# ChainSafe/halo2-verifier

Hardware: AMD Instinct MI355X
Metric: proofs verified/sec (BN254, k=14) (higher is better)
Workload: dtype u32 limbs (254-bit prime-field integers)

## Files before the change

### halo2_verifier_amd/csrc/bn254.hip.h

```cpp
#pragma once
#include <hip/hip_runtime.h>
#include <stdint.h>

#define H2V_HD __host__ __device__ inline
#define H2V_FN __host__ __device__ inline __attribute__((noinline))

namespace h2v {

#define H2V_LIMBS 9
#define H2V_LIMB_BITS 29
#define H2V_LIMB_MASK 0x1fffffffu

struct FqParams {
    static constexpr uint32_t INV29 = 0x04866389u;
    H2V_HD static constexpr uint32_t P(int i) {
        constexpr uint32_t p[8] = {0xd87cfd47u, 0x3c208c16u, 0x6871ca8du, 0x97816a91u, 0x8181585du, 0xb85045b6u, 0xe131a029u, 0x30644e72u};
        return p[i];
    }
    H2V_HD static constexpr uint32_t P29(int i) {
        constexpr uint32_t v[9] = {0x187cfd47u, 0x010460b6u, 0x1c72a34fu, 0x02d522d0u, 0x1585d978u, 0x02db40c0u, 0x00a6e141u, 0x0e5c2634u, 0x0030644eu};
        return v[i];
    }
    H2V_HD static constexpr uint32_t ONE(int i) {
        constexpr uint32_t v[9] = {0x157ccc21u, 0x141c2758u, 0x185230d3u, 0x014c0419u, 0x0aa36fb9u, 0x1d4240ceu, 0x11d54c07u, 0x052ac7a8u, 0x000dc836u};
        return v[i];
    }
    H2V_HD static constexpr uint32_t R2(int i) {
        constexpr uint32_t v[9] = {0x059bac10u, 0x0d1503a3u, 0x018016b8u, 0x10ab0ca8u, 0x02632639u, 0x02c0169fu, 0x169bfd53u, 0x11869d4cu, 0x002a11a6u};
        return v[i];
    }
    H2V_HD static constexpr uint32_t M256(int i) {
        constexpr uint32_t v[9] = {0x0f6b5c04u, 0x08ead878u, 0x1645525du, 0x1aefe9cdu, 0x09d605edu, 0x0483a115u, 0x0d08508bu, 0x0dba4804u, 0x001982b4u};
        return v[i];
    }
    H2V_HD static constexpr uint32_t K266(int i) {
// ... 323 lines not shown
        r.v[8] = (uint32_t)acc;
        return r;
    }
    __host__ __device__ __forceinline__ Fp sqr_inl() const {
        uint64_t acc = 0;
        uint32_t m[9], d[9];
        Fp r;
#pragma unroll
        for (int i = 0; i < 9; ++i) d[i] = v[i] << 1;
#pragma unroll
        for (int k = 0; k < 9; ++k) {
#pragma unroll
            for (int i = 0; 2 * i < k; ++i) acc += (uint64_t)d[i] * v[k - i];
            if (k % 2 == 0) acc += (uint64_t)v[k / 2] * v[k / 2];
#pragma unroll
            for (int i = 0; i < k; ++i) acc += (uint64_t)m[i] * PR::P29(k - i);
            m[k] = ((uint32_t)acc * PR::INV29) & H2V_LIMB_MASK;
            acc += (uint64_t)m[k] * PR::P29(0);
            acc >>= 29;
        }
#pragma unroll
        for (int k = 9; k < 17; ++k) {
#pragma unroll
            for (int i = k - 8; 2 * i < k; ++i) acc += (uint64_t)d[i] * v[k - i];
            if (k % 2 == 0) acc += (uint64_t)v[k / 2] * v[k / 2];
#pragma unroll
            for (int i = k - 8; i <= 8; ++i) acc += (uint64_t)m[i] * PR::P29(k - i);
            r.v[k - 9] = (uint32_t)acc & H2V_LIMB_MASK;
            acc >>= 29;
        }
        r.v[8] = (uint32_t)acc;
        return r;
    }
    H2V_FN static Fp mul(Fp a, Fp b) { return mul_inl(a, b); }
    H2V_FN static Fp sqr_fn(Fp a) { return a.sqr_inl(); }
    H2V_HD Fp operator*(const Fp& b) const { return mul(*this, b); }
    H2V_HD Fp sqr() const { return sqr_fn(*this); }

    H2V_HD static Fp from_raw(const uint32_t raw[8]) { Fp t; pack29(t.v, raw); return mul(t, r2()); }
    H2V_HD static Fp from_raw_unreduced(const uint32_t raw[8]) { return from_raw(raw); }
    H2V_HD static Fp from_mont256(const uint32_t m[8]) { Fp t, k; pack29(t.v, m); for (int i = 0; i < 9; ++i) k.v[i] = PR::K266(i); return mul(t, k); }
    H2V_HD void to_raw(uint32_t out[8]) const {
        Fp o = zero(); o.v[0] = 1;
        Fp r = mul(*this, o);
        uint32_t c[9]; r.canonical(c);
        unpack29(out, c);
    }
    H2V_HD static Fp from_u32(uint32_t x) { uint32_t raw[8] = {x, 0, 0, 0, 0, 0, 0, 0}; return from_raw(raw); }

    H2V_HD static bool from_bytes(const uint8_t b[32], Fp& out) {
        uint32_t raw[8];
        for (int i = 0; i < 8; ++i) raw[i] = (uint32_t)b[4 * i] | ((uint32_t)b[4 * i + 1] << 8) | ((uint32_t)b[4 * i + 2] << 16) | ((uint32_t)b[4 * i + 3] << 24);
        if (geq_p(raw)) return false;
        out = from_raw(raw);
        return true;
    }
    H2V_HD void to_bytes(uint8_t b[32]) const {
        uint32_t raw[8]; to_raw(raw);
        for (int i = 0; i < 8; ++i) { b[4 * i] = (uint8_t)raw[i]; b[4 * i + 1] = (uint8_t)(raw[i] >> 8); b[4 * i + 2] = (uint8_t)(raw[i] >> 16); b[4 * i + 3] = (uint8_t)(raw[i] >> 24); }
    }
    H2V_HD static Fp from_uniform_words(const uint32_t w[16]) {
        Fp lo = from_raw(w), hi = from_raw(w + 8), m256;
        for (int i = 0; i < 9; ++i) m256.v[i] = PR::M256(i);
        return lo + hi * m256;
    }

    H2V_FN Fp pow_u32(uint32_t e) const {
        Fp r = one();
// ... 42 lines not shown
```

### halo2_verifier_amd/csrc/curve.hip.h

```cpp
#pragma once
#include "bn254.hip.h"

namespace h2v {

static constexpr uint8_t G1_FLAG_IDENTITY = 0x80;
static constexpr uint8_t G1_FLAG_SIGN = 0x40;

struct G1A {
    Fq x, y;
    H2V_HD bool is_identity() const { return x.is_zero() && y.is_zero(); }
    H2V_HD static G1A identity() { G1A p; p.x = Fq::zero(); p.y = Fq::zero(); return p; }
    H2V_HD bool on_curve() const {
        if (is_identity()) return true;
        Fq three = Fq::from_u32(3);
        return y.sqr() == x.sqr() * x + three;
    }
};

struct G1J {
    Fq X, Y, Z;
    H2V_HD static G1J identity() { G1J p; p.X = Fq::zero(); p.Y = Fq::one(); p.Z = Fq::zero(); return p; }
    H2V_HD bool is_identity() const { return Z.is_zero(); }
    H2V_HD static G1J from_affine(const G1A& a) {
        if (a.is_identity()) return identity();
        G1J p; p.X = a.x; p.Y = a.y; p.Z = Fq::one(); return p;
    }
    H2V_HD G1J neg() const { G1J r = *this; r.Y = Y.neg(); return r; }
};

H2V_FN G1J g1_dbl(const G1J& p);
#define H2V_M(a, b) Fq::mul_inl((a), (b))
#define H2V_S(a) (a).sqr_inl()
__host__ __device__ __forceinline__ Fq g1_minus_eight() {
    const Fq k = {{0x1d9096cdu, 0x022be75eu, 0x12c66350u, 0x1e1f47a4u, 0x0b760e9fu, 0x1e7fbbcfu, 0x134a4383u, 0x01be3557u, 0x0022eb3au}};
    return k;
}
__host__ __device__ __forceinline__ G1J g1_dbl_inl(const G1J& p) {
    if (p.is_identity()) return p;
    const Fq A = H2V_S(p.X), B = H2V_S(p.Y), XB = H2V_M(p.X, B), C = H2V_S(B);
    const Fq E = Fq::lazy_add2(A, A), F = H2V_S(E), D = Fq::lazy_dbl(Fq::lazy_dbl(XB));
    int64_t acc[9];
#pragma unroll
    for (int l = 0; l < 9; ++l) acc[l] = (int64_t)F.v[l] + (int64_t)Fq::KP29(9, l) - 2 * (int64_t)D.v[l];
    G1J r;
    r.X = Fq::from_wide(acc);
    r.Y = Fq::dot2_inl(E, Fq::lazy_sub(D, r.X), C, g1_minus_eight());
    r.Z = H2V_M(Fq::lazy_dbl(p.Y), p.Z);
    return r;
}

__host__ __device__ __forceinline__ bool g1_madd_fast(G1J& acc, const G1A& q) {
    if (q.is_identity()) return true;
    if (acc.is_identity()) { acc.X = q.x; acc.Y = q.y; acc.Z = Fq::one(); return true; }
    const Fq Z1Z1 = H2V_S(acc.Z);
    const Fq U2 = H2V_M(q.x, Z1Z1), S2 = H2V_M(H2V_M(q.y, acc.Z), Z1Z1);
    const Fq H = Fq::lazy_sub(U2, acc.X), H2 = Fq::lazy_dbl(H), I = H2V_S(H2);
    if (I.is_zero()) return false;
    const Fq B = Fq::lazy_neg2(acc.Y), rr = Fq::lazy_add2(B, S2);
    const Fq X3 = Fq::dot2_inl(rr, rr, I, Fq::template lazy_lin<8, 1, 2>(H, acc.X));
    const Fq W = Fq::dot2_inl(rr, acc.X, H, B);
    acc.Y = Fq::dot2_inl(I, W, rr, Fq::lazy_neg(X3));
    acc.Z = H2V_M(acc.Z, H2);
    acc.X = X3;
    return true;
}
__host__ __device__ __forceinline__ bool g1_add_fast(G1J& acc, const G1J& q) {
    if (q.is_identity()) return true;
    if (acc.is_identity()) { acc.X = q.X; acc.Y = q.Y; acc.Z = q.Z; return true; }
    const Fq Z1Z1 = H2V_S(acc.Z), Z2Z2 = H2V_S(q.Z);
    const Fq U1 = H2V_M(acc.X, Z2Z2), U2 = H2V_M(q.X, Z1Z1);
    const Fq H = Fq::lazy_sub(U2, U1), H2 = Fq::lazy_dbl(H), I = H2V_S(H2);
    if (I.is_zero()) return false;
    const Fq S1 = H2V_M(H2V_M(acc.Y, q.Z), Z2Z2), S2 = H2V_M(H2V_M(q.Y, acc.Z), Z1Z1);
    const Fq B = Fq::lazy_neg2(S1), rr = Fq::lazy_add2(B, S2);
    const Fq X3 = Fq::dot2_inl(rr, rr, I, Fq::template lazy_lin<8, 1, 2>(H, U1));
    const Fq W = Fq::dot2_inl(rr, U1, H, B);
    acc.Y = Fq::dot2_inl(I, W, rr, Fq::lazy_neg(X3));
    acc.Z = H2V_M(H2V_M(acc.Z, q.Z), H2);
    acc.X = X3;
    return true;
}
__host__ __device__ __forceinline__ G1J g1_add_inl(const G1J& p, const G1J& q) {
    G1J r = p;
    if (g1_add_fast(r, q)) return r;
    const Fq Z1Z1 = H2V_S(p.Z), Z2Z2 = H2V_S(q.Z);
    const Fq S1 = H2V_M(H2V_M(p.Y, q.Z), Z2Z2), S2 = H2V_M(H2V_M(q.Y, p.Z), Z1Z1);
    if (S1 == S2) return g1_dbl(r);
    return G1J::identity();
}

__host__ __device__ __forceinline__ G1J g1_add_affine_inl(const G1J& p, const G1A& q) {
    G1J r = p;
    if (g1_madd_fast(r, q)) return r;
    const Fq Z1Z1 = H2V_S(p.Z);
    const Fq S2 = H2V_M(H2V_M(q.y, p.Z), Z1Z1);
    if (p.Y == S2) return g1_dbl(r);
    return G1J::identity();
}

H2V_FN G1J g1_dbl(const G1J& p) { return g1_dbl_inl(p); }
__host__ __device__ __forceinline__ Fq g1_beta_times(const Fq& x) {
    const Fq beta = {{0x18ccb791u, 0x175b1c3au, 0x0b83d6e2u, 0x0e8ed071u, 0x1282bee2u, 0x04220e84u, 0x1fe4017fu, 0x15084d4au, 0x00169119u}};
    return Fq::mul_inl(x, beta);
}
__host__ __device__ __forceinline__ G1A g1_phi(const G1A& p) { G1A r; r.x = g1_beta_times(p.x); r.y = p.y; return r; }
H2V_FN G1J g1_add(const G1J& p, const G1J& q) { return g1_add_inl(p, q); }
H2V_FN G1J g1_add_affine(const G1J& p, const G1A& q) { return g1_add_affine_inl(p, q); }

H2V_FN G1A g1_to_affine(const G1J& p) {
    if (p.is_identity()) return G1A::identity();
    Fq zi = p.Z.inv(), zi2 = zi.sqr();
    G1A a; a.x = p.X * zi2; a.y = p.Y * zi2 * zi;
    return a;
}

struct FqSqrtSchedule { uint8_t op[400]; int n; };
template <int W> constexpr FqSqrtSchedule fq_sqrt_schedule() {
    constexpr uint32_t e[8] = {0xb61f3f52u, 0x4f082305u, 0x5a1c72a3u, 0x65e05aa4u, 0xa0605617u, 0x6e14116du, 0xb84c680au, 0x0c19139cu};
    FqSqrtSchedule s{};
    s.n = 0;
    int i = 255;
    while (i >= 0 && !((e[i >> 5] >> (i & 31)) & 1)) --i;
    while (i >= 0) {
        if (!((e[i >> 5] >> (i & 31)) & 1)) { s.op[s.n++] = 0; --i; continue; }
        int l = i - (W - 1) < 0 ? 0 : i - (W - 1);
        while (!((e[l >> 5] >> (l & 31)) & 1)) ++l;
        uint32_t v = 0;
        for (int k = i; k >= l; --k) { v = (v << 1) | ((e[k >> 5] >> (k & 31)) & 1); s.op[s.n++] = 0; }
        s.op[s.n++] = (uint8_t)((v + 1) / 2);
        i = l - 1;
    }
    return s;
}
template <int W> __host__ __device__ inline __attribute__((noinline)) Fq fq_sqrt_candidate_w(const Fq& a) {
    constexpr FqSqrtSchedule S = fq_sqrt_schedule<W>();
    constexpr int T = 1 << (W - 1);
    Fq t[T];
    t[0] = a;
    const Fq a2 = a.sqr();
#pragma unroll
    for (int k = 1; k < T; ++k) t[k] = t[k - 1] * a2;
    Fq r = Fq::one();
    bool started = false;
#pragma unroll
    for (int k = 0; k < S.n; ++k) {
        if (S.op[k] == 0) { if (started) r = r.sqr(); }
        else { r = started ? r * t[S.op[k] - 1] : t[S.op[k] - 1]; started = true; }
    }
    return r;
}
H2V_FN Fq fq_sqrt_candidate(const Fq& a) { return fq_sqrt_candidate_w<4>(a); }

struct FqSqrtRuns { uint8_t nsq[160]; uint8_t idx[160]; int n; int first; };
template <int W> constexpr FqSqrtRuns fq_sqrt_runs() {
    constexpr FqSqrtSchedule S = fq_sqrt_schedule<W>();
    FqSqrtRuns r{};
    r.n = 0; r.first = -1;
    int pending = 0;
    for (int k = 0; k < S.n; ++k) {
        if (S.op[k] == 0) { if (r.first >= 0) ++pending; continue; }
        if (r.first < 0) { r.first = S.op[k] - 1; continue; }
        r.nsq[r.n] = (uint8_t)pending; r.idx[r.n] = (uint8_t)(S.op[k] - 1); ++r.n; pending = 0;
    }
    if (pending) { r.nsq[r.n] = (uint8_t)pending; r.idx[r.n] = 255; ++r.n; }
    return r;
}
#if defined(__HIPCC__)
__device__ __constant__ const FqSqrtRuns fq_sqrt_runs_w3 = fq_sqrt_runs<3>();
__device__ __forceinline__ Fq fq_sqrt_candidate_loop_w3(const Fq& a) {
    Fq t0 = a;
    const Fq a2 = a.sqr_inl();
    const Fq t1 = Fq::mul_inl(t0, a2), t2 = Fq::mul_inl(t1, a2), t3 = Fq::mul_inl(t2, a2);
    auto pick = [&](uint32_t i) -> Fq {
        Fq s;
#pragma unroll
        for (int l = 0; l < H2V_LIMBS; ++l) s.v[l] = i == 0 ? t0.v[l] : (i == 1 ? t1.v[l] : (i == 2 ? t2.v[l] : t3.v[l]));
        return s;
    };
    Fq r = pick((uint32_t)fq_sqrt_runs_w3.first);
    const int n = fq_sqrt_runs_w3.n;
#pragma unroll 1
    for (int k = 0; k < n; ++k) {
        const uint32_t nsq = fq_sqrt_runs_w3.nsq[k], idx = fq_sqrt_runs_w3.idx[k];
#pragma unroll 1
        for (uint32_t i = 0; i < nsq; ++i) r = r.sqr_inl();
        if (idx == 0u) r = Fq::mul_inl(r, t0);
        else if (idx == 1u) r = Fq::mul_inl(r, t1);
        else if (idx == 2u) r = Fq::mul_inl(r, t2);
        else if (idx == 3u) r = Fq::mul_inl(r, t3);
    }
    return r;
}
#endif

H2V_FN bool g1_decompress(const uint8_t in[32], G1A& out) {
    uint8_t tmp[32];
    for (int i = 0; i < 32; ++i) tmp[i] = in[i];
    bool is_inf = tmp[31] & G1_FLAG_IDENTITY, sign = tmp[31] & G1_FLAG_SIGN;
    tmp[31] &= 0x3f;
    Fq x;
    if (!Fq::from_bytes(tmp, x)) return false;
    if (is_inf) {
        if (!x.is_zero() || sign) return false;
        out = G1A::identity();
        return true;
    }
    Fq rhs = x.sqr() * x + Fq::from_u32(3);
    Fq y = fq_sqrt_candidate(rhs);
    if (y.sqr() != rhs) return false;
    if (y.is_odd() != sign) y = y.neg();
    out.x = x; out.y = y;
    return true;
}

template <int S> __device__ __forceinline__ Fq quad_bcast(const Fq& v) {
    Fq r;
#pragma unroll
    for (int l = 0; l < H2V_LIMBS; ++l) r.v[l] = (uint32_t)__builtin_amdgcn_mov_dpp((int)v.v[l], S * 0x55, 0xf, 0xf, true);
    return r;
}
__device__ __forceinline__ Fq fq_sel(bool c, const Fq& a, const Fq& b) {
    Fq r;
#pragma unroll
    for (int l = 0; l < H2V_LIMBS; ++l) r.v[l] = c ? a.v[l] : b.v[l];
    return r;
}
__device__ __forceinline__ void g1_dbl_quad(G1J& p, uint32_t r) {
    const Fq Y2 = Fq::lazy_dbl(p.Y);
    const Fq p1 = Fq::mul_inl(fq_sel(r == 0, p.X, fq_sel(r == 1, p.Y, Y2)), fq_sel(r == 0, p.X, fq_sel(r == 1, p.Y, p.Z)));
    const Fq A = quad_bcast<0>(p1), B = quad_bcast<1>(p1), Z3 = quad_bcast<2>(p1);
    const Fq E = Fq::lazy_add2(A, A);
    const Fq p2 = Fq::mul_inl(fq_sel(r == 0, B, fq_sel(r == 1, p.X, E)), fq_sel(r == 2, E, B));
    const Fq C = quad_bcast<0>(p2), XB = quad_bcast<1>(p2), F = quad_bcast<2>(p2);
    const Fq D = Fq::lazy_dbl(Fq::lazy_dbl(XB));
    int64_t acc[9];
#pragma unroll
    for (int l = 0; l < 9; ++l) acc[l] = (int64_t)F.v[l] + (int64_t)Fq::KP29(9, l) - 2 * (int64_t)D.v[l];
    p.X = Fq::from_wide(acc);
    p.Y = Fq::dot2_inl(E, Fq::lazy_sub(D, p.X), C, g1_minus_eight());
    p.Z = Z3;
}
template <class Slot> __device__ __forceinline__ G1J msm_horner_quad(const Slot* __restrict__ src, uint32_t items, uint32_t dbl, uint32_t r) {
    G1J acc = src[items - 1].p;
    for (int w = (int)items - 2; w >= 0; --w) {
        const G1J cur = src[w].p;
#pragma unroll 1
        for (uint32_t i = 0; i < dbl; ++i) g1_dbl_quad(acc, r);
        acc = g1_add_inl(acc, cur);
    }
    return acc;
}

}
```

### halo2_verifier_amd/csrc/msm.hip

```cpp
#include "../../include/h2v.h"
#include <hip/hip_ext.h>
#include "batch.h"

namespace h2v {

#define MSM_LDS_SORT_MAX_TERMS 16384u
#define MSM_SORT_THREADS 512u
#define MSM_CHUNK_MIN 16u
#define MSM_CHUNK_MAX 64u
#define MSM_ACC_LANES_PER_ROUND 196608u
#define MSM_CHUNK_SMALL 4u
#define MSM_SHORT_LIST 98304u
__host__ __device__ __forceinline__ uint32_t msm_chunk_len(uint32_t E, uint32_t R) {
    if (E <= MSM_SHORT_LIST) return MSM_CHUNK_SMALL;
    if (E <= R * MSM_CHUNK_MIN) return MSM_CHUNK_MIN;
    const uint32_t k = (uint32_t)(((uint64_t)E + (uint64_t)R * MSM_CHUNK_MAX - 1) / ((uint64_t)R * MSM_CHUNK_MAX));
    const uint32_t c = (uint32_t)(((uint64_t)E + (uint64_t)k * R - 1) / ((uint64_t)k * R));
    return c < MSM_CHUNK_MIN ? MSM_CHUNK_MIN : c;
}
static inline uint32_t msm_accumulate_blocks(size_t max_entries, size_t R) {
    size_t lanes;
    if (max_entries <= R * MSM_CHUNK_MIN)
        lanes = std::max<size_t>((max_entries + MSM_CHUNK_MIN - 1) / MSM_CHUNK_MIN, (std::min<size_t>(max_entries, MSM_SHORT_LIST) + MSM_CHUNK_SMALL - 1) / MSM_CHUNK_SMALL);
    else lanes = (max_entries + R * MSM_CHUNK_MAX - 1) / (R * MSM_CHUNK_MAX) * R;
// ... 638 lines not shown
                                             const uint32_t* __restrict__ lists, G1JSlot* __restrict__ bucket_pts, uint32_t nb, const MsmSeg& g, uint32_t first_block) {
    const uint32_t n_heavy = counts[nb], t = threadIdx.x;
    const uint32_t CH = msm_chunk_len(counts[nb + 1], g.lanes_round);
    for (uint32_t h = blockIdx.x - first_block; h < n_heavy; h += MSM_FIXUP_HEAVY_BLOCKS) {
        const uint32_t b = lists[nb - 1 - h];
        const uint32_t cnt = counts[b], off = msm_bin_start(g, offsets, b);
        const uint32_t i0 = off / CH, i1 = (off + cnt - 1) / CH;
        G1J acc = G1J::identity();
        for (uint32_t i = i0 + t; i <= i1; i += 64) acc = g1_add(acc, msm_piece_src(partial, i, i0, off, CH)->p);
        for (uint32_t d = 32; d > 0; d >>= 1) {
            G1J other;
            uint32_t* dst = reinterpret_cast<uint32_t*>(&other);
            const uint32_t* src = reinterpret_cast<const uint32_t*>(&acc);
#pragma unroll
            for (uint32_t k = 0; k < sizeof(G1J) / 4; ++k) dst[k] = (uint32_t)__shfl_down((int)src[k], d, 64);
            acc = g1_add(acc, other);
        }
        if (t == 0) bucket_pts[b] = acc;
    }
}
__global__ void __launch_bounds__(64) msm_fixup(const uint32_t* __restrict__ counts, const uint32_t* __restrict__ offsets, const G1JSlot* __restrict__ partial,
                                                const uint32_t* __restrict__ lists, G1JSlot* __restrict__ bucket_pts, uint32_t nb, MsmSeg g) {
    __shared__ G1J team_acc[64];
    if (blockIdx.x < MSM_FIXUP_TEAM_BLOCKS) { msm_fixup_team(counts, offsets, partial, lists, bucket_pts, nb, g, team_acc); return; }
    if (blockIdx.x < MSM_FIXUP_TEAM_BLOCKS + MSM_FIXUP_HEAVY_BLOCKS) { msm_fixup_heavy(counts, offsets, partial, lists, bucket_pts, nb, g, MSM_FIXUP_TEAM_BLOCKS); return; }
    const uint32_t k = (blockIdx.x - MSM_FIXUP_TEAM_BLOCKS - MSM_FIXUP_HEAVY_BLOCKS) * blockDim.x + threadIdx.x;
    if (k >= counts[nb + 2]) return;
    const uint32_t b = lists[k];
    const uint32_t cnt = counts[b], off = msm_bin_start(g, offsets, b);
    const uint32_t CH = msm_chunk_len(counts[nb + 1], g.lanes_round);
    const uint32_t i0 = off / CH, i1 = (off + cnt - 1) / CH;
    G1J acc = msm_piece_src(partial, i0, i0, off, CH)->p;
    bool ok = true;
    for (uint32_t i = i0 + 1; i <= i1 && ok; ++i) ok = g1_add_fast(acc, msm_piece_src(partial, i, i0, off, CH)->p);
    if (!ok) { msm_fixup_slow(partial, i0, i1, off, CH, bucket_pts + b); return; }
    bucket_pts[b] = acc;
}
#define MSM_WIN_SLOTS 5
__device__ __noinline__ void g1_add_to(G1J* dst, const G1J* a, const G1J* b) { const G1J x = *a, y = *b; *dst = g1_add_inl(x, y); }
__device__ __noinline__ void g1_dbl_to(G1J* dst, const G1J* a) { const G1J x = *a; *dst = g1_dbl_inl(x); }

__global__ void __launch_bounds__(MSM_WIN_THREADS) msm_window(const G1JSlot* __restrict__ bucket_pts, const uint32_t* __restrict__ counts, G1JSlot* __restrict__ window_sums, MsmPlan p,
                                                              uint32_t n_windows, uint32_t wpw, uint32_t slots) {
    __builtin_amdgcn_s_setprio(3);
    extern __shared__ G1J win_lds[];
    const uint32_t T = blockDim.x / wpw, sub = threadIdx.x / T, t = threadIdx.x % T;
    const uint32_t widx = blockIdx.x * wpw + sub;
    const bool live = widx < n_windows;
    G1J* mine = win_lds + (size_t)sub * slots * T;
    G1J* run = mine + t;
    G1J* sum = mine + T + t;
    G1J* scaled = mine + 2 * T + t;
    G1J* red = mine + 2 * T;
    const uint32_t slice = (p.buckets + T - 1) / T;
    const uint32_t lo = live ? min(p.buckets, t * slice) : 0, hi = live ? min(p.buckets, lo + slice) : 0;
    *run = G1J::identity(); *sum = G1J::identity();
    const G1JSlot* bp = bucket_pts + (size_t)widx * p.buckets;
    const uint32_t* cn = counts + (size_t)widx * p.buckets;
    for (uint32_t b = hi; b > lo; --b) {
        if (cn[b - 1]) g1_add_to(run, run, &bp[b - 1].p);
        g1_add_to(sum, sum, run);
    }
    if ((slice & (slice - 1)) == 0 && T > 1 && slots >= MSM_WIN_SLOTS) {
        G1J* run2 = mine + 3 * T + t;
        G1J* run3 = mine + 4 * T + t;
        if (lo < hi && t > 0) {
            g1_dbl_to(run2, run);
// ... 40 lines not shown
        const uint32_t* src = reinterpret_cast<const uint32_t*>(&mine_sum);
#pragma unroll
        for (uint32_t k = 0; k < sizeof(G1J) / 4; ++k) dst[k] = (uint32_t)__shfl_down((int)src[k], d, 64);
        if ((t & (W - 1)) + d >= W) other = G1J::identity();
        *scaled = other;
        g1_add_to(sum, sum, scaled);
    }
    __syncthreads();
    if ((t & (W - 1)) == 0) red[t >> 6] = *sum;
    __syncthreads();
    if (t == 0) {
        for (uint32_t wv = 1; wv < (T >> 6); ++wv) g1_add_to(&red[0], &red[0], &red[wv]);
        if (live) window_sums[widx] = red[0];
    }
}

__global__ void __launch_bounds__(64) msm_final(const G1JSlot* __restrict__ window_sums, const MsmProblem* __restrict__ prs, uint32_t count, MsmPlan p) {
    __builtin_amdgcn_s_setprio(3);
    const uint32_t t = blockIdx.x * blockDim.x + threadIdx.x, q = t >> 2, r = t & 3u;
    if (q >= count) return;
    G1J acc = G1J::identity();
    if (prs[q].n) acc = msm_horner_quad(window_sums + (size_t)q * p.windows, p.windows, p.c, r);
    if (r == 0) *prs[q].out = acc;
}
__global__ void __launch_bounds__(64) msm_final_parts(const G1JSlot* __restrict__ window_sums, const MsmProblem* __restrict__ prs, uint32_t count, MsmPlan p,
                                                      uint32_t parts, uint32_t wpp, G1JSlot* __restrict__ out, G1JSlot* __restrict__ ready) {
    __builtin_amdgcn_s_setprio(3);
    const uint32_t t = blockIdx.x * blockDim.x + threadIdx.x, quad = t >> 2, r = t & 3u;
    if (quad >= count * parts) return;
    const uint32_t q = quad / parts, j = quad % parts, lo = j * wpp, hi = min(p.windows, lo + wpp);
    G1J acc = G1J::identity();
    if (prs[q].n && lo < hi) acc = msm_horner_quad(window_sums + (size_t)q * p.windows + lo, hi - lo, p.c, r);
    if (r == 0) out[quad] = acc;
    if (r == 0) { ready[quad].p.X = Fq::mul_inl(acc.X, acc.Z); ready[quad].p.Y = acc.Y; }
    if (r == 1) ready[quad].p.Z = Fq::mul_inl(acc.Z.sqr_inl(), acc.Z);
}
__global__ void __launch_bounds__(64) msm_combine_parts(const G1JSlot* __restrict__ pieces, const MsmProblem* __restrict__ prs, uint32_t count, uint32_t parts, uint32_t shift) {
    const uint32_t t = blockIdx.x * blockDim.x + threadIdx.x, q = t >> 2, r = t & 3u;
    if (q >= count) return;
    const G1J acc = msm_horner_quad(pieces + (size_t)q * parts, parts, shift, r);
    if (r == 0) *prs[q].out = acc;
}

__global__ void __launch_bounds__(64) msm_merge_windows(const G1JSlot* __restrict__ sub_sums, const MsmProblem* __restrict__ parents, uint32_t n_parents, uint32_t windows,
                                                        G1JSlot* __restrict__ merged) {
    const uint32_t team = (blockIdx.x * blockDim.x + threadIdx.x) >> 3, r = threadIdx.x & 7u;
    const bool live = team < n_parents * windows;
    const uint32_t q = live ? team / windows : 0, w = live ? team % windows : 0;
    const uint32_t first = parents[q].sub_first, cnt = live ? parents[q].sub_count : 0;
    G1J acc = G1J::identity();
    for (uint32_t k = r; k < cnt; k += 8) acc = g1_add(acc, sub_sums[(size_t)(first + k) * windows + w].p);
    for (uint32_t d = 4; d > 0; d >>= 1) {
        G1J other;
        uint32_t* dst = reinterpret_cast<uint32_t*>(&other);
        const uint32_t* src = reinterpret_cast<const uint32_t*>(&acc);
#pragma unroll
        for (uint32_t k = 0; k < sizeof(G1J) / 4; ++k) dst[k] = (uint32_t)__shfl_down((int)src[k], d, 8);
        acc = g1_add(acc, other);
    }
    if (live && r == 0) merged[(size_t)q * windows + w] = acc;
}

__global__ void msm_set_problems(MsmProblemChunk ch, uint32_t count, MsmProblem* __restrict__ dst) {
    uint32_t i = threadIdx.x;
    if (i < count) dst[i] = ch.p[i];
}

static MsmProblem msm_problem_slice(const MsmProblem& q, uint32_t first, uint32_t len) {
// ... 166 lines not shown
```

### halo2_verifier_amd/csrc/verify_kernels.hip

```cpp
#include "../../include/h2v.h"
#include "batch.h"
#include <atomic>

namespace h2v {

__global__ void __launch_bounds__(64, 4) k_decompress(const uint8_t* __restrict__ proofs, uint32_t proof_len, const uint32_t* __restrict__ point_offsets,
                                                   uint32_t np, uint32_t n_main_points, uint32_t n, G1A* __restrict__ pts, G1A* __restrict__ phi, uint8_t* __restrict__ ycanon,
                                                   int* __restrict__ status) {
    const uint32_t t_raw = blockIdx.x * blockDim.x + threadIdx.x;
    const uint32_t t = min(t_raw, n * np - 1);
    uint32_t p = t / np, slot = t % np;
    const uint4* src = reinterpret_cast<const uint4*>(proofs + (size_t)p * proof_len + point_offsets[slot]);
    const uint4 lo = src[0], hi = src[1];
    uint32_t w[8] = {lo.x, lo.y, lo.z, lo.w, hi.x, hi.y, hi.z, hi.w};
    const bool is_inf = (w[7] >> 24) & G1_FLAG_IDENTITY, sign = (w[7] >> 24) & G1_FLAG_SIGN;
    w[7] &= 0x3fffffffu;
    G1A a = G1A::identity();
    bool ok = !Fq::geq_p(w);
    uint32_t yraw[8] = {0, 0, 0, 0, 0, 0, 0, 0};
    if (ok) {
        const Fq x = Fq::from_raw(w);
        if (is_inf) ok = false;
        else {
            const Fq three = {{FqParams::ONE(0), FqParams::ONE(1), FqParams::ONE(2), FqParams::ONE(3), FqParams::ONE(4), FqParams::ONE(5), FqParams::ONE(6), FqParams::ONE(7), FqParams::ONE(8)}};
            const Fq rhs = x.sqr() * x + (three + three + three);
            Fq y = fq_sqrt_candidate_loop_w3(rhs);
            if (y.sqr() != rhs) ok = false;
            else {
                y.to_raw(yraw);
                uint32_t nz = 0;
#pragma unroll
                for (int i = 0; i < 8; ++i) nz |= yraw[i];
                if ((bool)(yraw[0] & 1u) != sign && nz) {
                    y = y.neg();
                    uint64_t borrow = 0;
#pragma unroll
                    for (int i = 0; i < 8; ++i) { const uint64_t d = (uint64_t)FqParams::P(i) - yraw[i] - borrow; yraw[i] = (uint32_t)d; borrow = (d >> 32) & 1u; }
                }
                a.x = x; a.y = y;
            }
        }
    }
    if (!ok) { status_set(status, p, slot < n_main_points ? H2V_DEV_ST_TRANSCRIPT : H2V_DEV_ST_OPENING); a = G1A::identity(); for (int i = 0; i < 8; ++i) yraw[i] = 0; }
    __shared__ uint32_t out_lds[64 * 18];
    const uint32_t lane = threadIdx.x, t0 = blockIdx.x * blockDim.x, live = min(64u, n * np - t0);
    const uint32_t* av = reinterpret_cast<const uint32_t*>(&a);
#pragma unroll
    for (int i = 0; i < 18; ++i) out_lds[lane * 18 + i] = av[i];
    __syncthreads();
    uint32_t* dp = reinterpret_cast<uint32_t*>(pts + t0);
#pragma unroll
    for (int i = 0; i < 18; ++i) { const uint32_t k = i * 64 + lane; if (k < live * 18) dp[k] = out_lds[k]; }
    __syncthreads();
    a.x = g1_beta_times(a.x);
#pragma unroll
    for (int i = 0; i < 9; ++i) out_lds[lane * 18 + i] = av[i];
    __syncthreads();
    dp = reinterpret_cast<uint32_t*>(phi + t0);
#pragma unroll
    for (int i = 0; i < 18; ++i) { const uint32_t k = i * 64 + lane; if (k < live * 18) dp[k] = out_lds[k]; }
    __syncthreads();
#pragma unroll
    for (int i = 0; i < 8; ++i) out_lds[lane * 8 + i] = yraw[i];
    __syncthreads();
    uint32_t* dy = reinterpret_cast<uint32_t*>(ycanon + (size_t)t0 * 32);
#pragma unroll
    for (int i = 0; i < 8; ++i) { const uint32_t k = i * 64 + lane; if (k < live * 8) dy[k] = out_lds[k]; }
}

__global__ void __launch_bounds__(256) k_check_scalars(const uint8_t* __restrict__ proofs, uint32_t proof_len, const uint32_t* __restrict__ scalar_offsets,
                                                       uint32_t ns, const uint8_t* __restrict__ inst, uint32_t ninst, uint32_t n, int* __restrict__ status) {
    uint32_t t = blockIdx.x * blockDim.x + threadIdx.x;
    uint32_t per = ns + ninst;
    if (t >= n * per) return;
    uint32_t p = t / per, i = t % per;
    const uint8_t* b = i < ns ? proofs + (size_t)p * proof_len + scalar_offsets[i] : inst + ((size_t)p * ninst + (i - ns)) * 32;
    const uint32_t top = ((uintptr_t)b & 3u) == 0 ? *reinterpret_cast<const uint32_t*>(b + 28)
// ... 365 lines not shown
        } else {
            const uint32_t* q = reinterpret_cast<const uint32_t*>(glob) + (size_t)s * H2V_LIMBS * n + p;
#pragma unroll
            for (int l = 0; l < H2V_LIMBS; ++l) r.v[l] = q[(size_t)l * n];
        }
        return r;
    }
    __device__ __forceinline__ void store(uint32_t s, const Fr& v) const {
        if (s < lds_slots) {
            uint32_t* q = lds + (size_t)s * H2V_LIMBS * 64 + lane;
#pragma unroll
            for (int l = 0; l < H2V_LIMBS; ++l) q[l * 64] = v.v[l];
        } else {
            uint32_t* q = reinterpret_cast<uint32_t*>(glob) + (size_t)s * H2V_LIMBS * n + p;
#pragma unroll
            for (int l = 0; l < H2V_LIMBS; ++l) q[(size_t)l * n] = v.v[l];
        }
    }
};

template <bool TWO> __device__ __forceinline__ void frvm_run(const FrvmArgs& a, const VmInstr* __restrict__ code, uint32_t n_code, const SlotFile& sf, uint32_t p, bool live) {
    const uint32_t n = a.n;
    Fr last = Fr::zero(); uint32_t last_d = 0xffffffffu;
    auto slot = [&](uint32_t x) -> Fr { return x == last_d ? last : sf.load(x); };
    auto opnd = [&](uint32_t x) -> Fr { return (x & VM_CONST_OPERAND) ? a.consts[x & ~VM_CONST_OPERAND] : slot(x); };
    auto put = [&](uint32_t d, const Fr& v) { sf.store(d, v); last = v; last_d = d; };
    VmInstr nx = code[0];
    for (uint32_t pc = 0; pc < n_code; ++pc) {
        const VmInstr in = nx;
        nx = code[pc + 1 < n_code ? pc + 1 : pc];
        switch (in.op) {
            case OP_BARRIER: if (TWO) __syncthreads(); last_d = 0xffffffffu; break;
            case OP_CONST: put(in.d, a.consts[in.a]); break;
            case OP_MUL: put(in.d, Fr::mul_inl(opnd(in.a), opnd(in.b))); break;
            case OP_ADD: put(in.d, opnd(in.a) + opnd(in.b)); break;
            case OP_SUB: put(in.d, opnd(in.a) - opnd(in.b)); break;
            case OP_NEG: put(in.d, slot(in.a).neg()); break;
            case OP_INV: {
                Fr v = slot(in.a);
                if (live && v.is_zero()) status_set(a.status, p, H2V_DEV_ST_PANIC);
                put(in.d, v.inv());
                break;
            }
            case OP_POW: put(in.d, slot(in.a).pow_u32(in.b)); break;
            case OP_SQRN: {
                Fr v = slot(in.a);
                for (uint32_t i = 0; i < in.b; ++i) v = v.sqr();
                put(in.d, v);
                break;
            }
            case OP_LOAD_SCALAR: put(in.d, fr_from_le32(a.proofs + (size_t)p * a.proof_len + a.scalar_offsets[in.a])); break;
            case OP_LOAD_INST: put(in.d, fr_from_le32(a.inst + ((size_t)p * a.ninst + in.a) * 32)); break;
            case OP_LOAD_CHAL: put(in.d, a.chal[(size_t)in.a * n + p]); break;
            case OP_LOAD_INSTEVAL: put(in.d, a.insteval[(size_t)in.a * n + p]); break;
            case OP_LOAD_MULT: put(in.d, a.mult[p]); break;
            case OP_STORE_MSM: {
                uint32_t raw[8];
                slot(in.a).to_raw(raw);
                bool bad = status_get(a.status, p) != 0;
                uint32_t* dst = a.msm_scal + ((size_t)p * a.np + in.b) * 8;
                if (live) for (int i = 0; i < 8; ++i) dst[i] = bad ? 0u : raw[i];
                break;
            }
            case OP_STORE_GUARD: {
                uint32_t raw[8];
                slot(in.a).to_raw(raw);
                uint32_t* dst = a.guard_scal + ((size_t)p * a.n_guard + in.b) * 8;
// ... 189 lines not shown
```

Measured before the change: 11.23 million.

## Use inline-asm v_mad_u64_u32 chains for Montgomery field mul, sqr and dot2

Adds column-wise Montgomery multiply, square, dot2 and a fused square-plus-product built from hand-written v_mad_u64_u32 accumulate chains in inline assembly, with the modulus limbs passed as scalar operands. The curve formulas, sqrt, the MSM finalisation and the scalar VM multiply now use these paths, and madd/add switch their rr*rr dot2 to the fused square form. The aim is to keep one 64-bit accumulator flowing through fused multiply-adds instead of letting the compiler emit separate multiply and add-with-carry sequences. The bucket-merge loop keeps the old path, and the decompress LDS buffer is enlarged, which may reduce occupancy. Inline asm limits compiler scheduling and register allocation and depends on every needed MadRun specialisation being present.

```diff
diff --git a/halo2_verifier_amd/csrc/bn254.hip.h b/halo2_verifier_amd/csrc/bn254.hip.h
--- a/halo2_verifier_amd/csrc/bn254.hip.h
+++ b/halo2_verifier_amd/csrc/bn254.hip.h
@@ -1,6 +1,8 @@
 #pragma once
 #include <hip/hip_runtime.h>
 #include <stdint.h>
+#include <utility>
+#include "field_chain.hip.h"
 
 #define H2V_HD __host__ __device__ inline
 #define H2V_FN __host__ __device__ inline __attribute__((noinline))
@@ -390,8 +392,121 @@
         r.v[8] = (uint32_t)acc;
         return r;
     }
-    H2V_FN static Fp mul(Fp a, Fp b) { return mul_inl(a, b); }
-    H2V_FN static Fp sqr_fn(Fp a) { return a.sqr_inl(); }
+#if defined(__HIP_DEVICE_COMPILE__)
+    template <int K, int NV> __device__ __forceinline__ static void chain_col(uint64_t& acc, uint32_t (&m)[9], Fp& r, const uint32_t* x, const uint32_t* y) {
+        constexpr int lo = K < 9 ? 0 : K - 8, ns = K < 9 ? K : 17 - K;
+        if constexpr (K == 0) {
+            acc = 0;
+#pragma unroll
+            for (int i = 0; i < NV; ++i) acc += (uint64_t)x[i] * y[i];
+        } else {
+            uint32_t mm[ns], q[ns];
+#pragma unroll
+            for (int j = 0; j < ns; ++j) { mm[j] = m[lo + j]; q[j] = PR::P29(K - lo - j); }
+            MadRun<NV, ns>::run(acc, x, y, mm, q);
+        }
+        if constexpr (K < 9) {
+            m[K] = ((uint32_t)acc * PR::INV29) & H2V_LIMB_MASK;
+            acc += (uint64_t)m[K] * PR::P29(0);
+        } else r.v[K - 9] = (uint32_t)acc & H2V_LIMB_MASK;
+        acc >>= 29;
+    }
+    template <int K> __device__ __forceinline__ static void mul_col(uint64_t& acc, uint32_t (&m)[9], Fp& r, const Fp& a, const Fp& b) {
+        constexpr int lo = K < 9 ? 0 : K - 8, n = K < 9 ? K + 1 : 17 - K;
+        uint32_t x[n], y[n];
+#pragma unroll
+        for (int j = 0; j < n; ++j) { x[j] = a.v[lo + j]; y[j] = b.v[K - lo - j]; }
+        chain_col<K, n>(acc, m, r, x, y);
+    }
+    template <int K> __device__ __forceinline__ static void dot2_col(uint64_t& acc, uint32_t (&m)[9], Fp& r, const Fp& a0, const Fp& b0, const Fp& a1, const Fp& b1) {
+        constexpr int lo = K < 9 ? 0 : K - 8, n = K < 9 ? K + 1 : 17 - K;
+        uint32_t x[2 * n], y[2 * n];
+#pragma unroll
+        for (int j = 0; j < n; ++j) { x[2 * j] = a0.v[lo + j]; y[2 * j] = b0.v[K - lo - j]; x[2 * j + 1] = a1.v[lo + j]; y[2 * j + 1] = b1.v[K - lo - j]; }
+        chain_col<K, 2 * n>(acc, m, r, x, y);
+    }
+    template <int K> __device__ __forceinline__ static void sqr_col(uint64_t& acc, uint32_t (&m)[9], Fp& r, const uint32_t (&d)[9], const Fp& a) {
+        constexpr int lo = K < 9 ? 0 : K - 8, off = (K + 1) / 2 - lo, n = off + (K % 2 == 0 ? 1 : 0);
+        uint32_t x[n], y[n];
+#pragma unroll
+        for (int j = 0; j < off; ++j) { x[j] = d[lo + j]; y[j] = a.v[K - lo - j]; }
+        if constexpr (K % 2 == 0) { x[off] = a.v[K / 2]; y[off] = a.v[K / 2]; }
+        chain_col<K, n>(acc, m, r, x, y);
+    }
+    template <int K> __device__ __forceinline__ static void sqdot_col(uint64_t& acc, uint32_t (&m)[9], Fp& r, const uint32_t (&d)[9], const Fp& a, const Fp& a1, const Fp& b1) {
+        constexpr int lo = K < 9 ? 0 : K - 8, off = (K + 1) / 2 - lo, nsq = off + (K % 2 == 0 ? 1 : 0), n = K < 9 ? K + 1 : 17 - K;
+        uint32_t x[nsq + n], y[nsq + n];
+#pragma unroll
+        for (int j = 0; j < off; ++j) { x[j] = d[lo + j]; y[j] = a.v[K - lo - j]; }
+        if constexpr (K % 2 == 0) { x[off] = a.v[K / 2]; y[off] = a.v[K / 2]; }
+#pragma unroll
+        for (int j = 0; j < n; ++j) { x[nsq + j] = a1.v[lo + j]; y[nsq + j] = b1.v[K - lo - j]; }
+        chain_col<K, nsq + n>(acc, m, r, x, y);
+    }
+    template <int... K> __device__ __forceinline__ static Fp mul_cols(const Fp& a, const Fp& b, std::integer_sequence<int, K...>) {
+        uint64_t acc; uint32_t m[9]; Fp r;
+        (mul_col<K>(acc, m, r, a, b), ...);
+        r.v[8] = (uint32_t)acc;
+        return r;
+    }
+    template <int... K> __device__ __forceinline__ static Fp dot2_cols(const Fp& a0, const Fp& b0, const Fp& a1, const Fp& b1, std::integer_sequence<int, K...>) {
+        uint64_t acc; uint32_t m[9]; Fp r;
+        (dot2_col<K>(acc, m, r, a0, b0, a1, b1), ...);
+        r.v[8] = (uint32_t)acc;
+        return r;
+    }
+    template <int... K> __device__ __forceinline__ static Fp sqr_cols(const Fp& a, std::integer_sequence<int, K...>) {
+        uint64_t acc; uint32_t m[9], d[9]; Fp r;
+#pragma unroll
+        for (int i = 0; i < 9; ++i) d[i] = a.v[i] << 1;
+        (sqr_col<K>(acc, m, r, d, a), ...);
+        r.v[8] = (uint32_t)acc;
+        return r;
+    }
+    template <int... K> __device__ __forceinline__ static Fp sqdot_cols(const Fp& a, const Fp& a1, const Fp& b1, std::integer_sequence<int, K...>) {
+        uint64_t acc; uint32_t m[9], d[9]; Fp r;
+#pragma unroll
+        for (int i = 0; i < 9; ++i) d[i] = a.v[i] << 1;
+        (sqdot_col<K>(acc, m, r, d, a, a1, b1), ...);
+        r.v[8] = (uint32_t)acc;
+        return r;
+    }
+#endif
+    __host__ __device__ __forceinline__ static Fp mul_chain(const Fp& a, const Fp& b) {
+#if defined(__HIP_DEVICE_COMPILE__)
+        return mul_cols(a, b, std::make_integer_sequence<int, 17>());
+#else
+        return mul_inl(a, b);
+#endif
+    }
+    __host__ __device__ __forceinline__ static Fp dot2_chain(const Fp& a0, const Fp& b0, const Fp& a1, const Fp& b1) {
+#if defined(__HIP_DEVICE_COMPILE__)
+        return dot2_cols(a0, b0, a1, b1, std::make_integer_sequence<int, 17>());
+#else
+        return dot2_inl(a0, b0, a1, b1);
+#endif
+    }
+    __host__ __device__ __forceinline__ Fp sqr_chain() const {
+#if defined(__HIP_DEVICE_COMPILE__)
+        return sqr_cols(*this, std::make_integer_sequence<int, 17>());
+#else
+        return sqr_inl();
+#endif
+    }
+    __host__ __device__ __forceinline__ static Fp sqdot_inl(const Fp& a, const Fp& a1, const Fp& b1) { return dot2_inl(a, a, a1, b1); }
+    __host__ __device__ __forceinline__ static Fp sqdot_chain(const Fp& a, const Fp& a1, const Fp& b1) {
+#if defined(__HIP_DEVICE_COMPILE__)
+        return sqdot_cols(a, a1, b1, std::make_integer_sequence<int, 17>());
+#else
+        return sqdot_inl(a, a1, b1);
+#endif
+    }
+    template <bool CHAIN> __host__ __device__ __forceinline__ static Fp mul_as(const Fp& a, const Fp& b) { if constexpr (CHAIN) return mul_chain(a, b); else return mul_inl(a, b); }
+    template <bool CHAIN> __host__ __device__ __forceinline__ static Fp dot2_as(const Fp& a0, const Fp& b0, const Fp& a1, const Fp& b1) { if constexpr (CHAIN) return dot2_chain(a0, b0, a1, b1); else return dot2_inl(a0, b0, a1, b1); }
+    template <bool CHAIN> __host__ __device__ __forceinline__ static Fp sqdot_as(const Fp& a, const Fp& a1, const Fp& b1) { if constexpr (CHAIN) return sqdot_chain(a, a1, b1); else return sqdot_inl(a, a1, b1); }
+    template <bool CHAIN> __host__ __device__ __forceinline__ Fp sqr_as() const { if constexpr (CHAIN) return sqr_chain(); else return sqr_inl(); }
+    H2V_FN static Fp mul(Fp a, Fp b) { return mul_chain(a, b); }
+    H2V_FN static Fp sqr_fn(Fp a) { return a.sqr_chain(); }
     H2V_HD Fp operator*(const Fp& b) const { return mul(*this, b); }
     H2V_HD Fp sqr() const { return sqr_fn(*this); }
 
diff --git a/halo2_verifier_amd/csrc/curve.hip.h b/halo2_verifier_amd/csrc/curve.hip.h
--- a/halo2_verifier_amd/csrc/curve.hip.h
+++ b/halo2_verifier_amd/csrc/curve.hip.h
@@ -29,13 +29,15 @@
 };
 
 H2V_FN G1J g1_dbl(const G1J& p);
-#define H2V_M(a, b) Fq::mul_inl((a), (b))
-#define H2V_S(a) (a).sqr_inl()
+#define H2V_M(a, b) Fq::template mul_as<CHAIN>((a), (b))
+#define H2V_S(a) (a).template sqr_as<CHAIN>()
+#define H2V_D(...) Fq::template dot2_as<CHAIN>(__VA_ARGS__)
+#define H2V_SD(...) Fq::template sqdot_as<CHAIN>(__VA_ARGS__)
 __host__ __device__ __forceinline__ Fq g1_minus_eight() {
     const Fq k = {{0x1d9096cdu, 0x022be75eu, 0x12c66350u, 0x1e1f47a4u, 0x0b760e9fu, 0x1e7fbbcfu, 0x134a4383u, 0x01be3557u, 0x0022eb3au}};
     return k;
 }
-__host__ __device__ __forceinline__ G1J g1_dbl_inl(const G1J& p) {
+template <bool CHAIN = true> __host__ __device__ __forceinline__ G1J g1_dbl_inl(const G1J& p) {
     if (p.is_identity()) return p;
     const Fq A = H2V_S(p.X), B = H2V_S(p.Y), XB = H2V_M(p.X, B), C = H2V_S(B);
     const Fq E = Fq::lazy_add2(A, A), F = H2V_S(E), D = Fq::lazy_dbl(Fq::lazy_dbl(XB));
@@ -44,12 +46,12 @@
     for (int l = 0; l < 9; ++l) acc[l] = (int64_t)F.v[l] + (int64_t)Fq::KP29(9, l) - 2 * (int64_t)D.v[l];
     G1J r;
     r.X = Fq::from_wide(acc);
-    r.Y = Fq::dot2_inl(E, Fq::lazy_sub(D, r.X), C, g1_minus_eight());
+    r.Y = H2V_D(E, Fq::lazy_sub(D, r.X), C, g1_minus_eight());
     r.Z = H2V_M(Fq::lazy_dbl(p.Y), p.Z);
     return r;
 }
 
-__host__ __device__ __forceinline__ bool g1_madd_fast(G1J& acc, const G1A& q) {
+template <bool CHAIN = true> __host__ __device__ __forceinline__ bool g1_madd_fast(G1J& acc, const G1A& q) {
     if (q.is_identity()) return true;
     if (acc.is_identity()) { acc.X = q.x; acc.Y = q.y; acc.Z = Fq::one(); return true; }
     const Fq Z1Z1 = H2V_S(acc.Z);
@@ -57,14 +59,14 @@
     const Fq H = Fq::lazy_sub(U2, acc.X), H2 = Fq::lazy_dbl(H), I = H2V_S(H2);
     if (I.is_zero()) return false;
     const Fq B = Fq::lazy_neg2(acc.Y), rr = Fq::lazy_add2(B, S2);
-    const Fq X3 = Fq::dot2_inl(rr, rr, I, Fq::template lazy_lin<8, 1, 2>(H, acc.X));
-    const Fq W = Fq::dot2_inl(rr, acc.X, H, B);
-    acc.Y = Fq::dot2_inl(I, W, rr, Fq::lazy_neg(X3));
+    const Fq X3 = H2V_SD(rr, I, Fq::template lazy_lin<8, 1, 2>(H, acc.X));
+    const Fq W = H2V_D(rr, acc.X, H, B);
+    acc.Y = H2V_D(I, W, rr, Fq::lazy_neg(X3));
     acc.Z = H2V_M(acc.Z, H2);
     acc.X = X3;
     return true;
 }
-__host__ __device__ __forceinline__ bool g1_add_fast(G1J& acc, const G1J& q) {
+template <bool CHAIN = true> __host__ __device__ __forceinline__ bool g1_add_fast(G1J& acc, const G1J& q) {
     if (q.is_identity()) return true;
     if (acc.is_identity()) { acc.X = q.X; acc.Y = q.Y; acc.Z = q.Z; return true; }
     const Fq Z1Z1 = H2V_S(acc.Z), Z2Z2 = H2V_S(q.Z);
@@ -73,25 +75,25 @@
     if (I.is_zero()) return false;
     const Fq S1 = H2V_M(H2V_M(acc.Y, q.Z), Z2Z2), S2 = H2V_M(H2V_M(q.Y, acc.Z), Z1Z1);
     const Fq B = Fq::lazy_neg2(S1), rr = Fq::lazy_add2(B, S2);
-    const Fq X3 = Fq::dot2_inl(rr, rr, I, Fq::template lazy_lin<8, 1, 2>(H, U1));
-    const Fq W = Fq::dot2_inl(rr, U1, H, B);
-    acc.Y = Fq::dot2_inl(I, W, rr, Fq::lazy_neg(X3));
+    const Fq X3 = H2V_SD(rr, I, Fq::template lazy_lin<8, 1, 2>(H, U1));
+    const Fq W = H2V_D(rr, U1, H, B);
+    acc.Y = H2V_D(I, W, rr, Fq::lazy_neg(X3));
     acc.Z = H2V_M(H2V_M(acc.Z, q.Z), H2);
     acc.X = X3;
     return true;
 }
-__host__ __device__ __forceinline__ G1J g1_add_inl(const G1J& p, const G1J& q) {
+template <bool CHAIN = true> __host__ __device__ __forceinline__ G1J g1_add_inl(const G1J& p, const G1J& q) {
     G1J r = p;
-    if (g1_add_fast(r, q)) return r;
+    if (g1_add_fast<CHAIN>(r, q)) return r;
     const Fq Z1Z1 = H2V_S(p.Z), Z2Z2 = H2V_S(q.Z);
     const Fq S1 = H2V_M(H2V_M(p.Y, q.Z), Z2Z2), S2 = H2V_M(H2V_M(q.Y, p.Z), Z1Z1);
     if (S1 == S2) return g1_dbl(r);
     return G1J::identity();
 }
 
-__host__ __device__ __forceinline__ G1J g1_add_affine_inl(const G1J& p, const G1A& q) {
+template <bool CHAIN = true> __host__ __device__ __forceinline__ G1J g1_add_affine_inl(const G1J& p, const G1A& q) {
     G1J r = p;
-    if (g1_madd_fast(r, q)) return r;
+    if (g1_madd_fast<CHAIN>(r, q)) return r;
     const Fq Z1Z1 = H2V_S(p.Z);
     const Fq S2 = H2V_M(H2V_M(q.y, p.Z), Z1Z1);
     if (p.Y == S2) return g1_dbl(r);
@@ -101,7 +103,7 @@
 H2V_FN G1J g1_dbl(const G1J& p) { return g1_dbl_inl(p); }
 __host__ __device__ __forceinline__ Fq g1_beta_times(const Fq& x) {
     const Fq beta = {{0x18ccb791u, 0x175b1c3au, 0x0b83d6e2u, 0x0e8ed071u, 0x1282bee2u, 0x04220e84u, 0x1fe4017fu, 0x15084d4au, 0x00169119u}};
-    return Fq::mul_inl(x, beta);
+    return Fq::mul_chain(x, beta);
 }
 __host__ __device__ __forceinline__ G1A g1_phi(const G1A& p) { G1A r; r.x = g1_beta_times(p.x); r.y = p.y; return r; }
 H2V_FN G1J g1_add(const G1J& p, const G1J& q) { return g1_add_inl(p, q); }
@@ -167,10 +169,10 @@
 }
 #if defined(__HIPCC__)
 __device__ __constant__ const FqSqrtRuns fq_sqrt_runs_w3 = fq_sqrt_runs<3>();
-__device__ __forceinline__ Fq fq_sqrt_candidate_loop_w3(const Fq& a) {
+template <bool CHAIN = true> __device__ __forceinline__ Fq fq_sqrt_candidate_loop_w3(const Fq& a) {
     Fq t0 = a;
-    const Fq a2 = a.sqr_inl();
-    const Fq t1 = Fq::mul_inl(t0, a2), t2 = Fq::mul_inl(t1, a2), t3 = Fq::mul_inl(t2, a2);
+    const Fq a2 = H2V_S(a);
+    const Fq t1 = H2V_M(t0, a2), t2 = H2V_M(t1, a2), t3 = H2V_M(t2, a2);
     auto pick = [&](uint32_t i) -> Fq {
         Fq s;
 #pragma unroll
@@ -183,11 +185,11 @@
     for (int k = 0; k < n; ++k) {
         const uint32_t nsq = fq_sqrt_runs_w3.nsq[k], idx = fq_sqrt_runs_w3.idx[k];
 #pragma unroll 1
-        for (uint32_t i = 0; i < nsq; ++i) r = r.sqr_inl();
-        if (idx == 0u) r = Fq::mul_inl(r, t0);
-        else if (idx == 1u) r = Fq::mul_inl(r, t1);
-        else if (idx == 2u) r = Fq::mul_inl(r, t2);
-        else if (idx == 3u) r = Fq::mul_inl(r, t3);
+        for (uint32_t i = 0; i < nsq; ++i) r = H2V_S(r);
+        if (idx == 0u) r = H2V_M(r, t0);
+        else if (idx == 1u) r = H2V_M(r, t1);
+        else if (idx == 2u) r = H2V_M(r, t2);
+        else if (idx == 3u) r = H2V_M(r, t3);
     }
     return r;
 }
@@ -227,17 +229,17 @@
 }
 __device__ __forceinline__ void g1_dbl_quad(G1J& p, uint32_t r) {
     const Fq Y2 = Fq::lazy_dbl(p.Y);
-    const Fq p1 = Fq::mul_inl(fq_sel(r == 0, p.X, fq_sel(r == 1, p.Y, Y2)), fq_sel(r == 0, p.X, fq_sel(r == 1, p.Y, p.Z)));
+    const Fq p1 = Fq::mul_chain(fq_sel(r == 0, p.X, fq_sel(r == 1, p.Y, Y2)), fq_sel(r == 0, p.X, fq_sel(r == 1, p.Y, p.Z)));
     const Fq A = quad_bcast<0>(p1), B = quad_bcast<1>(p1), Z3 = quad_bcast<2>(p1);
     const Fq E = Fq::lazy_add2(A, A);
-    const Fq p2 = Fq::mul_inl(fq_sel(r == 0, B, fq_sel(r == 1, p.X, E)), fq_sel(r == 2, E, B));
+    const Fq p2 = Fq::mul_chain(fq_sel(r == 0, B, fq_sel(r == 1, p.X, E)), fq_sel(r == 2, E, B));
     const Fq C = quad_bcast<0>(p2), XB = quad_bcast<1>(p2), F = quad_bcast<2>(p2);
     const Fq D = Fq::lazy_dbl(Fq::lazy_dbl(XB));
     int64_t acc[9];
 #pragma unroll
     for (int l = 0; l < 9; ++l) acc[l] = (int64_t)F.v[l] + (int64_t)Fq::KP29(9, l) - 2 * (int64_t)D.v[l];
     p.X = Fq::from_wide(acc);
-    p.Y = Fq::dot2_inl(E, Fq::lazy_sub(D, p.X), C, g1_minus_eight());
+    p.Y = Fq::dot2_chain(E, Fq::lazy_sub(D, p.X), C, g1_minus_eight());
     p.Z = Z3;
 }
 template <class Slot> __device__ __forceinline__ G1J msm_horner_quad(const Slot* __restrict__ src, uint32_t items, uint32_t dbl, uint32_t r) {
diff --git a/halo2_verifier_amd/csrc/field_chain.hip.h b/halo2_verifier_amd/csrc/field_chain.hip.h
--- /dev/null
+++ b/halo2_verifier_amd/csrc/field_chain.hip.h
@@ -0,0 +1,73 @@
+#pragma once
+#include <stdint.h>
+#if defined(__HIP_DEVICE_COMPILE__)
+namespace h2v {
+#define H2V_MAD(x, y) "v_mad_u64_u32 %[c], vcc, %[" #x "], %[" #y "], %[c]\n\t"
+#define H2V_VV1 H2V_MAD(x0, y0)
+#define H2V_VV2 H2V_VV1 H2V_MAD(x1, y1)
+#define H2V_VV3 H2V_VV2 H2V_MAD(x2, y2)
+#define H2V_VV4 H2V_VV3 H2V_MAD(x3, y3)
+#define H2V_VV5 H2V_VV4 H2V_MAD(x4, y4)
+#define H2V_VV6 H2V_VV5 H2V_MAD(x5, y5)
+#define H2V_VV7 H2V_VV6 H2V_MAD(x6, y6)
+#define H2V_VV8 H2V_VV7 H2V_MAD(x7, y7)
+#define H2V_VV9 H2V_VV8 H2V_MAD(x8, y8)
+#define H2V_VV10 H2V_VV9 H2V_MAD(x9, y9)
+#define H2V_VV11 H2V_VV10 H2V_MAD(x10, y10)
+#define H2V_VV12 H2V_VV11 H2V_MAD(x11, y11)
+#define H2V_VV13 H2V_VV12 H2V_MAD(x12, y12)
+#define H2V_VV14 H2V_VV13 H2V_MAD(x13, y13)
+#define H2V_VV15 H2V_VV14 H2V_MAD(x14, y14)
+#define H2V_VV16 H2V_VV15 H2V_MAD(x15, y15)
+#define H2V_VV17 H2V_VV16 H2V_MAD(x16, y16)
+#define H2V_VV18 H2V_VV17 H2V_MAD(x17, y17)
+#define H2V_OV1 [x0] "v"(x[0]), [y0] "v"(y[0])
+#define H2V_OV2 H2V_OV1, [x1] "v"(x[1]), [y1] "v"(y[1])
+#define H2V_OV3 H2V_OV2, [x2] "v"(x[2]), [y2] "v"(y[2])
+#define H2V_OV4 H2V_OV3, [x3] "v"(x[3]), [y3] "v"(y[3])
+#define H2V_OV5 H2V_OV4, [x4] "v"(x[4]), [y4] "v"(y[4])
+#define H2V_OV6 H2V_OV5, [x5] "v"(x[5]), [y5] "v"(y[5])
+#define H2V_OV7 H2V_OV6, [x6] "v"(x[6]), [y6] "v"(y[6])
+#define H2V_OV8 H2V_OV7, [x7] "v"(x[7]), [y7] "v"(y[7])
+#define H2V_OV9 H2V_OV8, [x8] "v"(x[8]), [y8] "v"(y[8])
+#define H2V_OV10 H2V_OV9, [x9] "v"(x[9]), [y9] "v"(y[9])
+#define H2V_OV11 H2V_OV10, [x10] "v"(x[10]), [y10] "v"(y[10])
+#define H2V_OV12 H2V_OV11, [x11] "v"(x[11]), [y11] "v"(y[11])
+#define H2V_OV13 H2V_OV12, [x12] "v"(x[12]), [y12] "v"(y[12])
+#define H2V_OV14 H2V_OV13, [x13] "v"(x[13]), [y13] "v"(y[13])
+#define H2V_OV15 H2V_OV14, [x14] "v"(x[14]), [y14] "v"(y[14])
+#define H2V_OV16 H2V_OV15, [x15] "v"(x[15]), [y15] "v"(y[15])
+#define H2V_OV17 H2V_OV16, [x16] "v"(x[16]), [y16] "v"(y[16])
+#define H2V_OV18 H2V_OV17, [x17] "v"(x[17]), [y17] "v"(y[17])
+#define H2V_VS1 H2V_MAD(m0, q0)
+#define H2V_VS2 H2V_VS1 H2V_MAD(m1, q1)
+#define H2V_VS3 H2V_VS2 H2V_MAD(m2, q2)
+#define H2V_VS4 H2V_VS3 H2V_MAD(m3, q3)
+#define H2V_VS5 H2V_VS4 H2V_MAD(m4, q4)
+#define H2V_VS6 H2V_VS5 H2V_MAD(m5, q5)
+#define H2V_VS7 H2V_VS6 H2V_MAD(m6, q6)
+#define H2V_VS8 H2V_VS7 H2V_MAD(m7, q7)
+#define H2V_OS1 , [m0] "v"(m[0]), [q0] "s"(q[0])
+#define H2V_OS2 H2V_OS1, [m1] "v"(m[1]), [q1] "s"(q[1])
+#define H2V_OS3 H2V_OS2, [m2] "v"(m[2]), [q2] "s"(q[2])
+#define H2V_OS4 H2V_OS3, [m3] "v"(m[3]), [q3] "s"(q[3])
+#define H2V_OS5 H2V_OS4, [m4] "v"(m[4]), [q4] "s"(q[4])
+#define H2V_OS6 H2V_OS5, [m5] "v"(m[5]), [q5] "s"(q[5])
+#define H2V_OS7 H2V_OS6, [m6] "v"(m[6]), [q6] "s"(q[6])
+#define H2V_OS8 H2V_OS7, [m7] "v"(m[7]), [q7] "s"(q[7])
+template <int NV, int NS> struct MadRun;
+#define H2V_RUN(NV, NS)                                                                                                              \
+    template <> struct MadRun<NV, NS> {                                                                                              \
+        __device__ __forceinline__ static void run(uint64_t& c, const uint32_t* x, const uint32_t* y, const uint32_t* m, const uint32_t* q) { \
+            asm(H2V_VV##NV H2V_VS##NS : [c] "+v"(c) : H2V_OV##NV H2V_OS##NS : "vcc");                                                \
+        }                                                                                                                            \
+    };
+H2V_RUN(1, 1) H2V_RUN(1, 2) H2V_RUN(2, 1) H2V_RUN(2, 2) H2V_RUN(2, 3) H2V_RUN(2, 4) H2V_RUN(3, 2)
+H2V_RUN(3, 3) H2V_RUN(3, 4) H2V_RUN(3, 5) H2V_RUN(3, 6) H2V_RUN(4, 1) H2V_RUN(4, 2) H2V_RUN(4, 3)
+H2V_RUN(4, 4) H2V_RUN(4, 6) H2V_RUN(4, 7) H2V_RUN(4, 8) H2V_RUN(5, 4) H2V_RUN(5, 5) H2V_RUN(5, 8)
+H2V_RUN(6, 2) H2V_RUN(6, 3) H2V_RUN(6, 5) H2V_RUN(6, 6) H2V_RUN(7, 6) H2V_RUN(7, 7) H2V_RUN(8, 3)
+H2V_RUN(8, 4) H2V_RUN(8, 7) H2V_RUN(8, 8) H2V_RUN(9, 8) H2V_RUN(10, 4) H2V_RUN(10, 5) H2V_RUN(12, 5)
+H2V_RUN(12, 6) H2V_RUN(14, 6) H2V_RUN(14, 7) H2V_RUN(16, 7) H2V_RUN(16, 8) H2V_RUN(18, 8)
+H2V_RUN(3, 1) H2V_RUN(5, 2) H2V_RUN(5, 3) H2V_RUN(6, 4) H2V_RUN(8, 5) H2V_RUN(9, 5) H2V_RUN(9, 6) H2V_RUN(11, 6) H2V_RUN(11, 7) H2V_RUN(12, 7) H2V_RUN(12, 8) H2V_RUN(14, 8)
+}
+#endif
diff --git a/halo2_verifier_amd/csrc/msm.hip b/halo2_verifier_amd/csrc/msm.hip
--- a/halo2_verifier_amd/csrc/msm.hip
+++ b/halo2_verifier_amd/csrc/msm.hip
@@ -694,7 +694,7 @@
     const uint32_t i0 = off / CH, i1 = (off + cnt - 1) / CH;
     G1J acc = msm_piece_src(partial, i0, i0, off, CH)->p;
     bool ok = true;
-    for (uint32_t i = i0 + 1; i <= i1 && ok; ++i) ok = g1_add_fast(acc, msm_piece_src(partial, i, i0, off, CH)->p);
+    for (uint32_t i = i0 + 1; i <= i1 && ok; ++i) ok = g1_add_fast<false>(acc, msm_piece_src(partial, i, i0, off, CH)->p);
     if (!ok) { msm_fixup_slow(partial, i0, i1, off, CH, bucket_pts + b); return; }
     bucket_pts[b] = acc;
 }
@@ -801,8 +801,8 @@
     G1J acc = G1J::identity();
     if (prs[q].n && lo < hi) acc = msm_horner_quad(window_sums + (size_t)q * p.windows + lo, hi - lo, p.c, r);
     if (r == 0) out[quad] = acc;
-    if (r == 0) { ready[quad].p.X = Fq::mul_inl(acc.X, acc.Z); ready[quad].p.Y = acc.Y; }
-    if (r == 1) ready[quad].p.Z = Fq::mul_inl(acc.Z.sqr_inl(), acc.Z);
+    if (r == 0) { ready[quad].p.X = Fq::mul_chain(acc.X, acc.Z); ready[quad].p.Y = acc.Y; }
+    if (r == 1) ready[quad].p.Z = Fq::mul_chain(acc.Z.sqr_chain(), acc.Z);
 }
 __global__ void __launch_bounds__(64) msm_combine_parts(const G1JSlot* __restrict__ pieces, const MsmProblem* __restrict__ prs, uint32_t count, uint32_t parts, uint32_t shift) {
     const uint32_t t = blockIdx.x * blockDim.x + threadIdx.x, q = t >> 2, r = t & 3u;
diff --git a/halo2_verifier_amd/csrc/verify_kernels.hip b/halo2_verifier_amd/csrc/verify_kernels.hip
--- a/halo2_verifier_amd/csrc/verify_kernels.hip
+++ b/halo2_verifier_amd/csrc/verify_kernels.hip
@@ -4,6 +4,7 @@
 
 namespace h2v {
 
+#define K_DECOMPRESS_LDS_WORDS 2560
 __global__ void __launch_bounds__(64, 4) k_decompress(const uint8_t* __restrict__ proofs, uint32_t proof_len, const uint32_t* __restrict__ point_offsets,
                                                    uint32_t np, uint32_t n_main_points, uint32_t n, G1A* __restrict__ pts, G1A* __restrict__ phi, uint8_t* __restrict__ ycanon,
                                                    int* __restrict__ status) {
@@ -42,7 +43,7 @@
         }
     }
     if (!ok) { status_set(status, p, slot < n_main_points ? H2V_DEV_ST_TRANSCRIPT : H2V_DEV_ST_OPENING); a = G1A::identity(); for (int i = 0; i < 8; ++i) yraw[i] = 0; }
-    __shared__ uint32_t out_lds[64 * 18];
+    __shared__ uint32_t out_lds[K_DECOMPRESS_LDS_WORDS];
     const uint32_t lane = threadIdx.x, t0 = blockIdx.x * blockDim.x, live = min(64u, n * np - t0);
     const uint32_t* av = reinterpret_cast<const uint32_t*>(&a);
 #pragma unroll
@@ -474,7 +475,7 @@
         switch (in.op) {
             case OP_BARRIER: if (TWO) __syncthreads(); last_d = 0xffffffffu; break;
             case OP_CONST: put(in.d, a.consts[in.a]); break;
-            case OP_MUL: put(in.d, Fr::mul_inl(opnd(in.a), opnd(in.b))); break;
+            case OP_MUL: put(in.d, Fr::mul_chain(opnd(in.a), opnd(in.b))); break;
             case OP_ADD: put(in.d, opnd(in.a) + opnd(in.b)); break;
             case OP_SUB: put(in.d, opnd(in.a) - opnd(in.b)); break;
             case OP_NEG: put(in.d, slot(in.a).neg()); break;
```

Result: faster. 11.83 million (median of 6 runs) (+5.4%).
